# Aleph-Alpha/magma

Hardware: NVIDIA H100
Metric: image-caption samples/sec (fwd+bwd) (higher is better)
Workload: dtype bf16

## Files before the change

magma_b200/csrc/gemm.cu:

```cuda
#include <mutex>
#include <stdlib.h>

#include "gemm_common.cuh"

namespace mb200 {

template <int BN, bool A_MN, bool B_MN>
__global__ void __launch_bounds__(kThreads, 1)
gemm_wgmma_kernel(const __grid_constant__ CUtensorMap tmA, const __grid_constant__ CUtensorMap tmB,
                  const __grid_constant__ GemmKernelParams p) {
  using C_ = Cfg<BN>;
  constexpr int kStages = C_::kStages;

  extern __shared__ uint8_t smem_raw[];
  uint8_t* smem = reinterpret_cast<uint8_t*>((reinterpret_cast<uintptr_t>(smem_raw) + 1023) & ~uintptr_t(1023));
  uint8_t* smem_a = smem;
  uint8_t* smem_b = smem + kStages * C_::kABytes;
  float* epi_stage = reinterpret_cast<float*>(smem + kStages * C_::kStageBytes);
  uint64_t* full_bar = reinterpret_cast<uint64_t*>(smem + kStages * C_::kStageBytes + kEpiBytes);
  uint64_t* empty_bar = full_bar + kStages;

  const int wg = threadIdx.x >> 7;
  const int num_kb = (p.K + BK - 1) / BK;
  const int items = p.total_tiles * p.split_k;

  pdl_trigger();
  if (threadIdx.x == 0) {
    tma_prefetch_desc(&tmA);
    tma_prefetch_desc(&tmB);
    for (int s = 0; s < kStages; ++s) {
      mbar_init(&full_bar[s], 1);
      mbar_init(&empty_bar[s], 2);
    }
    mbar_fence_init();
  }
  __syncthreads();
  pdl_wait();

  if (wg == 0) {
    setmaxnreg_dec<40>();
    if (threadIdx.x == 0) {
      int stage = 0;
      uint32_t phase = 0;
      for (int w = blockIdx.x; w < items; w += gridDim.x) {
        const int t = w / p.split_k, ks = w - t * p.split_k;
        const int kb0 = ks * p.kb_per_split, kb1 = min(num_kb, kb0 + p.kb_per_split);
        const int tpb = p.tiles_m * p.tiles_n;
        const int z = t / tpb;
        const int r = t - z * tpb;
        const int m_blk = r % p.tiles_m;
        const int n_blk = r / p.tiles_m;
        const int z0 = z % p.nb0, z1 = z / p.nb0;
        for (int kb = kb0; kb < kb1; ++kb) {
          mbar_wait(&empty_bar[stage], phase ^ 1);
          mbar_expect_tx(&full_bar[stage], (uint32_t)C_::kStageBytes);
          uint8_t* sa = smem_a + stage * C_::kABytes;
          uint8_t* sb = smem_b + stage * C_::kBBytes;
          const int kc = kb * BK;
          if constexpr (A_MN) {
#pragma unroll
            for (int i = 0; i < BM / 64; ++i)
              tma_load_4d(sa + i * 8192, &tmA, &full_bar[stage], m_blk * BM + i * 64, kc, z0, z1);
          } else {
            tma_load_4d(sa, &tmA, &full_bar[stage], kc, m_blk * BM, z0, z1);
          }
          if constexpr (B_MN) {
#pragma unroll
            for (int i = 0; i < BN / 64; ++i)
              tma_load_4d(sb + i * 8192, &tmB, &full_bar[stage], n_blk * BN + i * 64, kc, z0, z1);
          } else {
            tma_load_4d(sb, &tmB, &full_bar[stage], kc, n_blk * BN, z0, z1);
          }
          if (++stage == kStages) {
            stage = 0;
            phase ^= 1;
          }
        }
      }
    }
  } else {
    setmaxnreg_inc<232>();
    const int cw = wg - 1;
    const bool leader = (threadIdx.x & 127) == 0;
    constexpr uint32_t b_lbo = B_MN ? 8192u : 0u;
    constexpr uint32_t a_kadv = A_MN ? 2048u : 32u, b_kadv = B_MN ? 2048u : 32u;
    const uint32_t a_off = (uint32_t)cw * 8192u;
    int stage = 0;
    uint32_t phase = 0;
    float acc[BN / 2];
    for (int w = blockIdx.x; w < items; w += gridDim.x) {
      const int t = w / p.split_k, ks = w - t * p.split_k;
      const int kb0 = ks * p.kb_per_split, kb1 = min(num_kb, kb0 + p.kb_per_split);
      const int tpb = p.tiles_m * p.tiles_n;
      const int z = t / tpb;
      const int r = t - z * tpb;
      const int m_blk = r % p.tiles_m;
      const int n_blk = r / p.tiles_m;
      const int z0 = z % p.nb0, z1 = z / p.nb0;
      int prev = -1;
      for (int kb = kb0; kb < kb1; ++kb) {
        mbar_wait(&full_bar[stage], phase);
        const uint32_t sa = smem_u32(smem_a + stage * C_::kABytes) + a_off;
        const uint32_t sb = smem_u32(smem_b + stage * C_::kBBytes);
        wgmma_fence();
#pragma unroll
        for (int k = 0; k < BK / WG_K; ++k) {
          const uint64_t da = make_smem_desc(sa + k * a_kadv, 0u, 1024);
          const uint64_t db = make_smem_desc(sb + k * b_kadv, b_lbo, 1024);
          wgmma_bf16<BN, A_MN ? 1 : 0, B_MN ? 1 : 0>(acc, da, db, (kb > kb0 || k > 0) ? 1u : 0u);
        }
        wgmma_commit();
        wgmma_wait<1>();
        if (prev >= 0 && leader) mbar_arrive(&empty_bar[prev]);
        prev = stage;
        if (++stage == kStages) {
          stage = 0;
          phase ^= 1;
        }
      }
      wgmma_wait<0>();
      if (prev >= 0 && leader) mbar_arrive(&empty_bar[prev]);
      const long long boff = (long long)z0 * p.c_bs0 + (long long)z1 * p.c_bs1;
      epi_tile<BN>(p, acc, epi_stage + cw * 64 * kEpiCols, 1 + cw, boff, m_blk * BM + cw * 64, n_blk * BN, ks);
    }
  }
}

__global__ void splitk_finalize_kernel(const GemmKernelParams p) {
  pdl_trigger();
  pdl_wait();
  const int ncol4 = (p.N + 3) >> 2;
  const long long total = (long long)p.M * ncol4;
  for (long long i = blockIdx.x * (long long)blockDim.x + threadIdx.x; i < total; i += (long long)gridDim.x * blockDim.x) {
    const int row = (int)(i / ncol4);
    const int col = (int)(i - (long long)row * ncol4) * 4;
    float v[4] = {0.f, 0.f, 0.f, 0.f};
    for (int ks = 0; ks < p.split_k; ++ks) {
      const float4 w4 = *reinterpret_cast<const float4*>(p.splitk_ws + ((long long)ks * p.M + row) * p.ld_ws + col);
      v[0] += w4.x;
      v[1] += w4.y;
      v[2] += w4.z;
      v[3] += w4.w;
    }
    epi_store4(p, 0, row, col, v);
  }
}

typedef CUresult (*PFN_encodeTiled)(CUtensorMap*, CUtensorMapDataType, cuuint32_t, void*, const cuuint64_t*,
                                    const cuuint64_t*, const cuuint32_t*, const cuuint32_t*, CUtensorMapInterleave,
                                    CUtensorMapSwizzle, CUtensorMapL2promotion, CUtensorMapFloatOOBfill);

static PFN_encodeTiled get_encode_fn() {
  static PFN_encodeTiled fn = nullptr;
  static std::once_flag once;
  std::call_once(once, [] {
    void* p = nullptr;
    cudaDriverEntryPointQueryResult qres;
    if (cudaGetDriverEntryPoint("cuTensorMapEncodeTiled", &p, cudaEnableDefault, &qres) == cudaSuccess &&
        qres == cudaDriverEntryPointSuccess)
      fn = reinterpret_cast<PFN_encodeTiled>(p);
  });
  return fn;
}

int make_operand_map(CUtensorMap* out, const mb200_operand& op, int rows, int K, int nb0, int nb1,
                            int box_rows) {
  PFN_encodeTiled enc = get_encode_fn();
  MB_REQUIRE(enc != nullptr, MB200_E_CUDA, "cuTensorMapEncodeTiled entry point unavailable");
  MB_REQUIRE((reinterpret_cast<uintptr_t>(op.ptr) & 15) == 0, MB200_E_ALIGN, "gemm operand pointer not 16B aligned");
  MB_REQUIRE(op.ld % 8 == 0, MB200_E_ALIGN, "gemm operand ld (%lld) must be a multiple of 8 elements",
             (long long)op.ld);
  MB_REQUIRE((nb0 == 1 || op.bs0 % 8 == 0) && (nb1 == 1 || op.bs1 % 8 == 0), MB200_E_ALIGN,
             "gemm operand batch strides must be multiples of 8 elements");
  cuuint64_t dims[4];
  cuuint64_t strides[3];
  cuuint32_t box[4];
  cuuint32_t estr[4] = {1, 1, 1, 1};
  if (!op.mn_major) {
    dims[0] = (cuuint64_t)K;
    dims[1] = (cuuint64_t)rows;
    box[0] = BK;
    box[1] = (cuuint32_t)box_rows;
  } else {
    dims[0] = (cuuint64_t)rows;
    dims[1] = (cuuint64_t)K;
    box[0] = 64;
    box[1] = BK;
  }
  dims[2] = (cuuint64_t)nb0;
  dims[3] = (cuuint64_t)nb1;
  box[2] = 1;
  box[3] = 1;
  strides[0] = (cuuint64_t)op.ld * 2;
  strides[1] = (cuuint64_t)(nb0 > 1 ? op.bs0 : op.ld) * 2;
  strides[2] = (cuuint64_t)(nb1 > 1 ? op.bs1 : op.ld) * 2;
  CUresult r = enc(out, CU_TENSOR_MAP_DATA_TYPE_BFLOAT16, 4, const_cast<void*>(op.ptr), dims, strides, box, estr,
                   CU_TENSOR_MAP_INTERLEAVE_NONE, CU_TENSOR_MAP_SWIZZLE_128B, CU_TENSOR_MAP_L2_PROMOTION_L2_256B,
                   CU_TENSOR_MAP_FLOAT_OOB_FILL_NONE);
  MB_REQUIRE(r == CUDA_SUCCESS, MB200_E_CUDA,
             "cuTensorMapEncodeTiled failed (%d): dims=(%llu,%llu,%llu,%llu) strides=(%llu,%llu,%llu) box=(%u,%u)",
             (int)r, (unsigned long long)dims[0], (unsigned long long)dims[1], (unsigned long long)dims[2],
             (unsigned long long)dims[3], (unsigned long long)strides[0], (unsigned long long)strides[1],
             (unsigned long long)strides[2], box[0], box[1]);
  return 0;
}

template <int BN, bool A_MN, bool B_MN>
static int launch_gemm(const CUtensorMap& tmA, const CUtensorMap& tmB, const GemmKernelParams& kp,
                       cudaStream_t stream) {
  auto kern = gemm_wgmma_kernel<BN, A_MN, B_MN>;
  static bool attr_set = false;
  if (!attr_set) {
    MB_CUDA(cudaFuncSetAttribute(kern, cudaFuncAttributeMaxDynamicSharedMemorySize, Cfg<BN>::kSmemBytes));
    attr_set = true;
  }
  const long long items = (long long)kp.total_tiles * kp.split_k;
  int grid = items < gemm_sms() ? (int)items : gemm_sms();
  {
    const double nb = (double)kp.total_tiles / ((double)kp.tiles_m * kp.tiles_n);
    const double flops = 2.0 * kp.M * (double)kp.N * kp.K * nb;
    const double bytes = nb * (2.0 * ((double)kp.M * kp.K + (double)kp.N * kp.K) + (kp.c_f32 ? 4.0 : 2.0) * kp.M * kp.N);
    GemmProfScope prof(stream, flops, bytes);
    MB_CUDA(launch_pdl(kern, dim3(grid), dim3(kThreads), Cfg<BN>::kSmemBytes, stream, tmA, tmB, kp));
  }
  count_launch();
  MB_CUDA(cudaGetLastError());
  return 0;
}

template <int BN>
static int dispatch_major(bool a_mn, bool b_mn, const CUtensorMap& tmA, const CUtensorMap& tmB,
                          const GemmKernelParams& kp, cudaStream_t s) {
  if (!a_mn && !b_mn) return launch_gemm<BN, false, false>(tmA, tmB, kp, s);
  if (!a_mn && b_mn) return launch_gemm<BN, false, true>(tmA, tmB, kp, s);
  if (a_mn && !b_mn) return launch_gemm<BN, true, false>(tmA, tmB, kp, s);
  return launch_gemm<BN, true, true>(tmA, tmB, kp, s);
}

static int dispatch_bn(int bn, bool a_mn, bool b_mn, const CUtensorMap& tmA, const CUtensorMap& tmB,
                       const GemmKernelParams& kp, cudaStream_t s) {
  switch (bn) {
    case 64: return dispatch_major<64>(a_mn, b_mn, tmA, tmB, kp, s);
    case 128: return dispatch_major<128>(a_mn, b_mn, tmA, tmB, kp, s);
    default: return dispatch_major<256>(a_mn, b_mn, tmA, tmB, kp, s);
  }
}

static int pick_bn(int M, int N, int batches) {
  if (N <= 64) return 64;
  const int tiles_m = (M + BM - 1) / BM;
  const int sms = num_sms();
  double best = 1e300;
  int best_bn = 256;
  const int cands[3] = {256, 128, 64};
  const double tile_cost[3] = {1.0, 0.55, 0.3};
  for (int i = 0; i < 3; ++i) {
    const int bn = cands[i];
    if (bn > 64 && N <= bn / 2) continue;
    const long long t = (long long)tiles_m * ((N + bn - 1) / bn) * batches;
    const long long waves = (t + sms - 1) / sms;
    const double cost = (double)waves * tile_cost[i];
    if (cost < best - 1e-12) {
      best = cost;
      best_bn = bn;
    }
  }
  return best_bn;
}

struct SmallPlan {
  int bn, split;
};
static SmallPlan plan_small_m(int N, int K, int M, size_t ws_bytes) {
  const int sms = num_sms();
  const int num_kb = (K + BK - 1) / BK;
  const double kHbmRate = 3.35e12, kItem = 4e-6, kFinalize = 4e-6;
  SmallPlan best{64, 1};
  double best_t = 1e300;
  const int cands[3] = {256, 128, 64};
  for (int i = 0; i < 3; ++i) {
    const int bn = cands[i];
    if (bn > 64 && N <= bn / 2) continue;
    const int tiles = (N + bn - 1) / bn;
    for (int split = 1; split <= 16; ++split) {
      if (split > 1) {
        if (num_kb / split < 8) break;
        if ((size_t)split * M * ((N + 3) / 4 * 4) * sizeof(float) > ws_bytes) break;
      }
      const int kb_per = (num_kb + split - 1) / split;
      const int eff_split = (num_kb + kb_per - 1) / kb_per;
      const long long items = (long long)tiles * eff_split;
      const long long waves = (items + sms - 1) / sms;
      const double active = (double)(items < sms ? items : sms);
      const double sm_rate = bn == 64 ? 40e9 : 50e9;
      const double rate = sm_rate < kHbmRate / active ? sm_rate : kHbmRate / active;
      const double t = kItem + waves * ((double)kb_per * bn * BK * 2 / rate) + (eff_split > 1 ? kFinalize : 0.0);
      if (t < best_t - 1e-12) {
        best_t = t;
        best = SmallPlan{bn, eff_split};
      }
    }
  }
  return best;
}

int gemm_impl(const mb200_gemm_args* a, cudaStream_t stream) {
  MB_REQUIRE(a != nullptr, MB200_E_ARG, "null gemm args");
  MB_REQUIRE(a->M > 0 && a->N > 0 && a->K > 0 && a->nb0 > 0 && a->nb1 > 0, MB200_E_SHAPE,
             "gemm: bad shape M=%d N=%d K=%d nb=(%d,%d)", a->M, a->N, a->K, a->nb0, a->nb1);
  MB_REQUIRE(a->c_dtype == MB200_BF16 || a->c_dtype == MB200_F32, MB200_E_DTYPE, "gemm: bad c_dtype %d", a->c_dtype);
  MB_REQUIRE(!(a->accumulate && a->c_dtype != MB200_F32), MB200_E_DTYPE, "gemm: accumulate needs f32 output");
  MB_REQUIRE(!(a->dact && !a->aux_in), MB200_E_ARG, "gemm: dact needs aux_in");
  const int celt = a->c_dtype == MB200_F32 ? 4 : 8;
  MB_REQUIRE((reinterpret_cast<uintptr_t>(a->C) & 15) == 0 && a->ldc % celt == 0, MB200_E_ALIGN,
             "gemm: C must be 16B aligned with ldc multiple of %d", celt);
  MB_REQUIRE((a->nb0 == 1 || a->c_bs0 % celt == 0) && (a->nb1 == 1 || a->c_bs1 % celt == 0), MB200_E_ALIGN,
             "gemm: C batch strides must be multiples of %d elements", celt);
  if (a->res1 || a->res2) MB_REQUIRE(a->ld_res % 8 == 0, MB200_E_ALIGN, "gemm: ld_res must be a multiple of 8");
  if (a->aux_in || a->aux_out)
    MB_REQUIRE(a->ldc % 8 == 0, MB200_E_ALIGN, "gemm: aux tensors share ldc, which must be a multiple of 8");
  int rc = check_arch();
  if (rc) return rc;

  int bn = a->force_bn ? a->force_bn : pick_bn(a->M, a->N, a->nb0 * a->nb1);
  MB_REQUIRE(bn == 64 || bn == 128 || bn == 256, MB200_E_ARG, "gemm: force_bn must be 64, 128 or 256");

  CUtensorMap tmA, tmB;
  const bool small_m = a->M <= 32 && a->A.mn_major == 0 && a->nb0 * a->nb1 == 1 && a->c_dtype == MB200_BF16;
  int plan_split = 1;
  if (small_m && !a->force_bn) {
    const SmallPlan pl = plan_small_m(a->N, a->K, a->M, a->splitk_ws ? (size_t)a->splitk_ws_bytes : 0);
    bn = pl.bn;
    plan_split = pl.split;
  }
  rc = make_operand_map(&tmA, a->A, a->M, a->K, a->nb0, a->nb1, BM);
  if (rc) return rc;

  GemmKernelParams kp;
  memset(&kp, 0, sizeof(kp));
  kp.M = a->M;
  kp.N = a->N;
  kp.K = a->K;
  kp.nb0 = a->nb0;
  kp.tiles_m = (a->M + BM - 1) / BM;
  kp.C = a->C;
  kp.ldc = a->ldc;
  kp.c_bs0 = a->c_bs0;
  kp.c_bs1 = a->c_bs1;
  kp.alpha = a->alpha;
  kp.act = a->act;
  kp.dact = a->dact;
  kp.accumulate = a->accumulate;
  kp.bias = reinterpret_cast<const bf16*>(a->bias);
  kp.aux_out = reinterpret_cast<bf16*>(a->aux_out);
  kp.aux_in = reinterpret_cast<const bf16*>(a->aux_in);
  kp.res1 = reinterpret_cast<const bf16*>(a->res1);
  kp.res2 = reinterpret_cast<const bf16*>(a->res2);
  kp.ld_res = a->ld_res;
  kp.epi_kind = EK_GENERIC;
  kp.c_f32 = a->c_dtype == MB200_F32 ? 1 : 0;
  kp.rope_tab = reinterpret_cast<const float2*>(a->rope_tab);
  kp.rope_mode = a->rope_tab ? a->rope_mode : 0;
  kp.rope_S = a->rope_S;
  kp.rope_hd = a->rope_hd;
  kp.rope_rot = a->rope_rot;
  kp.rope_ncols = a->rope_ncols;
  if (kp.rope_mode != 0)
    MB_REQUIRE(a->rope_S > 0 && a->rope_hd > 0 && a->rope_rot % 4 == 0 && a->rope_rot <= a->rope_hd &&
                   a->rope_hd % 4 == 0 && a->rope_ncols % 4 == 0,
               MB200_E_ARG, "gemm: bad rope epilogue parameters");

  const bool amn = a->A.mn_major != 0, bmn = a->B.mn_major != 0;
  kp.split_k = 1;
  kp.kb_per_split = (a->K + BK - 1) / BK;
  const bool split_mid = !small_m && a->splitk_ws && a->M <= 128 && a->nb0 * a->nb1 == 1 && a->K >= 8192 &&
                         a->N <= 8192 && !a->force_bn;
  const int bn_few = a->N >= 256 ? 256 : (a->N > 64 ? 128 : 64);
  const int tiles_m = kp.tiles_m;
  const bool split_few = !small_m && !split_mid && a->splitk_ws && a->M > 128 && a->nb0 * a->nb1 == 1 &&
                         a->K >= 2048 && !a->force_bn && 2 * tiles_m * ((a->N + bn_few - 1) / bn_few) <= num_sms();
  if (plan_split > 1 || split_mid || split_few) {
    const int bn_s = small_m ? bn : bn_few;
    const int tiles = (a->N + bn_s - 1) / bn_s;
    const int num_kb = (a->K + BK - 1) / BK;
    int split = plan_split;
    if (split_mid || split_few) {
      split = num_sms() / (tiles * tiles_m);
      if (split > num_kb / 4) split = num_kb / 4;
    }
    const long long ld_ws = (a->N + 3) / 4 * 4;
    while (split > 1 && (size_t)split * a->M * ld_ws * sizeof(float) > (size_t)a->splitk_ws_bytes) --split;
    if (split > 1) {
      const int kb_per = (num_kb + split - 1) / split;
      split = (num_kb + kb_per - 1) / kb_per;
      bn = bn_s;
      rc = make_operand_map(&tmB, a->B, a->N, a->K, a->nb0, a->nb1, bn);
      if (rc) return rc;
      kp.tiles_n = tiles;
      kp.total_tiles = tiles_m * tiles;
      kp.split_k = split;
      kp.kb_per_split = kb_per;
      kp.splitk_ws = reinterpret_cast<float*>(a->splitk_ws);
      kp.ld_ws = ld_ws;
      GemmKernelParams kg = kp;
      kg.epi_kind = EK_SPLITK;
      rc = dispatch_bn(bn, amn, bmn, tmA, tmB, kg, stream);
      if (rc) return rc;
      const long long n4 = (long long)a->M * ((a->N + 3) / 4);
      const int fgrid = (int)((n4 + 255) / 256 > 2048 ? 2048 : (n4 + 255) / 256);
      kp.alpha = 1.f;
      MB_CUDA(launch_pdl(splitk_finalize_kernel, dim3(fgrid), dim3(256), 0, stream, kp));
      count_launch();
      return 0;
    }
  }
  rc = make_operand_map(&tmB, a->B, a->N, a->K, a->nb0, a->nb1, bn);
  if (rc) return rc;
  kp.tiles_n = (a->N + bn - 1) / bn;
  kp.total_tiles = tiles_m * kp.tiles_n * a->nb0 * a->nb1;
  return dispatch_bn(bn, amn, bmn, tmA, tmB, kp, stream);
}

}

extern "C" int mb200_gemm(const mb200_gemm_args* args, void* stream) {
  return mb200::gemm_impl(args, reinterpret_cast<cudaStream_t>(stream));
}
```

magma_b200/csrc/gemm_common.cuh:

```cuda
#pragma once
#include "common.cuh"

namespace mb200 {

static constexpr int BM = 128;
static constexpr int BK = 64;
static constexpr int WG_K = 16;
static constexpr int kThreads = 384;
static constexpr int kEpiCols = 64;
static constexpr int kEpiBytes = BM * kEpiCols * 4;
static constexpr int kSmemBudget = 192 * 1024;

template <int BN>
struct Cfg {
  static constexpr int kABytes = BM * BK * 2;
  static constexpr int kBBytes = BN * BK * 2;
  static constexpr int kStageBytes = kABytes + kBBytes;
  static constexpr int kStagesRaw = kSmemBudget / kStageBytes;
  static constexpr int kStages = kStagesRaw > 8 ? 8 : kStagesRaw;
  static constexpr int kSmemBytes = kStages * kStageBytes + kEpiBytes + 1024  + 256 ;
  static_assert(kSmemBytes <= 227 * 1024, "GEMM shared memory exceeds the sm_90 per-block limit");
};

struct GemmKernelParams {
  int M, N, K;
  int nb0;
  int tiles_m, tiles_n, total_tiles;
  void* C;
  long long ldc, c_bs0, c_bs1;
  float alpha;
  int act, dact, accumulate;
  const bf16* bias;
  bf16* aux_out;
  const bf16* aux_in;
  const bf16* res1;
  const bf16* res2;
  long long ld_res;
  const float2* rope_tab;
  int rope_mode;
  int rope_S, rope_hd, rope_rot, rope_ncols;
  int epi_kind;
  int c_f32;
  int split_k, kb_per_split;
  float* splitk_ws;
  long long ld_ws;
};

__device__ __forceinline__ float2 bf16x2_to_f32(uint32_t u) {
  return __bfloat1622float2(*reinterpret_cast<const __nv_bfloat162*>(&u));
}
__device__ __forceinline__ uint32_t f32x2_to_bf16(float a, float b) {
  __nv_bfloat162 h = __floats2bfloat162_rn(a, b);
  return *reinterpret_cast<uint32_t*>(&h);
}

__device__ __forceinline__ void ld_bf16x4(const bf16* src, int n, float (&v)[4]) {
  if (n == 4 && (reinterpret_cast<uintptr_t>(src) & 7) == 0) {
    uint32_t u0, u1;
    asm volatile("ld.global.nc.v2.u32 {%0, %1}, [%2];" : "=r"(u0), "=r"(u1) : "l"(src));
    const float2 a = bf16x2_to_f32(u0), b = bf16x2_to_f32(u1);
    v[0] = a.x;
    v[1] = a.y;
    v[2] = b.x;
    v[3] = b.y;
  } else {
#pragma unroll
    for (int e = 0; e < 4; ++e) v[e] = e < n ? __bfloat162float(src[e]) : 0.f;
  }
}
__device__ __forceinline__ void st_bf16x4(bf16* dst, int n, const float (&v)[4]) {
  if (n == 4 && (reinterpret_cast<uintptr_t>(dst) & 7) == 0) {
    *reinterpret_cast<uint2*>(dst) = make_uint2(f32x2_to_bf16(v[0], v[1]), f32x2_to_bf16(v[2], v[3]));
  } else {
#pragma unroll
    for (int e = 0; e < 4; ++e)
      if (e < n) dst[e] = __float2bfloat16(v[e]);
  }
}

__device__ __forceinline__ void named_bar_sync(int id, int nthreads) {
  asm volatile("bar.sync %0, %1;" ::"r"(id), "r"(nthreads) : "memory");
}

enum { EK_GENERIC = 0, EK_SPLITK };

__device__ __forceinline__ void epi_store4(const GemmKernelParams& p, long long boff, int row, int col, float (&v)[4]) {
  const int n = min(4, p.N - col);
  if (p.bias) {
    float b[4];
    ld_bf16x4(p.bias + col, n, b);
#pragma unroll
    for (int e = 0; e < 4; ++e) v[e] += b[e];
  }
  if (p.rope_mode != 0 && col < p.rope_ncols) {
    const int dim = col % p.rope_hd;
    if (dim < p.rope_rot) {
      const float2* tp = p.rope_tab + (long long)(row % p.rope_S) * (p.rope_rot >> 1) + (dim >> 1);
      const float2 cs0 = __ldg(tp), cs1 = __ldg(tp + 1);
      const float sg = p.rope_mode > 0 ? 1.f : -1.f;
      const float a0 = v[0], a1 = v[1], a2 = v[2], a3 = v[3];
      v[0] = a0 * cs0.x - a1 * cs0.y * sg;
      v[1] = a1 * cs0.x + a0 * cs0.y * sg;
      v[2] = a2 * cs1.x - a3 * cs1.y * sg;
      v[3] = a3 * cs1.x + a2 * cs1.y * sg;
    }
  }
  const long long coff = boff + (long long)row * p.ldc + col;
  if (p.aux_out) st_bf16x4(p.aux_out + coff, n, v);
#pragma unroll
  for (int e = 0; e < 4; ++e) {
    if (p.act == MB200_ACT_GELU_NEW) v[e] = gelu_new_f(v[e]);
    else if (p.act == MB200_ACT_QUICK_GELU) v[e] = quick_gelu_f(v[e]);
    else if (p.act == MB200_ACT_RELU) v[e] = fmaxf(v[e], 0.f);
  }
  if (p.dact) {
    float a[4];
    ld_bf16x4(p.aux_in + coff, n, a);
#pragma unroll
    for (int e = 0; e < 4; ++e) v[e] = p.dact == MB200_DACT_GELU_NEW ? v[e] * gelu_new_grad_f(a[e]) : (a[e] > 0.f ? v[e] : 0.f);
  }
  const long long roff = boff + (long long)row * p.ld_res + col;
  if (p.res1) {
    float r[4];
    ld_bf16x4(p.res1 + roff, n, r);
#pragma unroll
    for (int e = 0; e < 4; ++e) v[e] += r[e];
  }
  if (p.res2) {
    float r[4];
    ld_bf16x4(p.res2 + roff, n, r);
#pragma unroll
    for (int e = 0; e < 4; ++e) v[e] += r[e];
  }
  if (p.act == MB200_ACT_RELU_POST) {
#pragma unroll
    for (int e = 0; e < 4; ++e) v[e] = fmaxf(v[e], 0.f);
  }
  if (p.c_f32) {
    float* dst = reinterpret_cast<float*>(p.C) + coff;
    if (n == 4) {
      float4 o = make_float4(v[0], v[1], v[2], v[3]);
      if (p.accumulate) {
        const float4 old = *reinterpret_cast<const float4*>(dst);
        o.x += old.x;
        o.y += old.y;
        o.z += old.z;
        o.w += old.w;
      }
      *reinterpret_cast<float4*>(dst) = o;
    } else {
#pragma unroll
      for (int e = 0; e < 4; ++e)
        if (e < n) dst[e] = p.accumulate ? dst[e] + v[e] : v[e];
    }
  } else {
    st_bf16x4(reinterpret_cast<bf16*>(p.C) + coff, n, v);
  }
}

template <int BN>
__device__ __forceinline__ void epi_tile(const GemmKernelParams& p, const float (&acc)[BN / 2], float* stage,
                                         int bar_id, long long boff, int row0, int col0, int ks) {
  const int wt = threadIdx.x & 127;
  const int fr = (wt >> 5) * 16 + ((wt & 31) >> 2);
  const int fq = wt & 3;
  const int pr = wt >> 4, pc = wt & 15;
  const int nch = min(BN / kEpiCols, (p.N - col0 + kEpiCols - 1) / kEpiCols);
#pragma unroll 1
  for (int ch = 0; ch < nch; ++ch) {
#pragma unroll
    for (int c = 0; c < BN / kEpiCols; ++c) {
      if (c != ch) continue;
#pragma unroll
      for (int jj = 0; jj < 8; ++jj) {
        const int j = c * 8 + jj;
#pragma unroll
        for (int h = 0; h < 2; ++h) {
          const int r = fr + 8 * h;
          const int q = (2 * jj + (fq >> 1)) ^ ((r & 3) << 1);
          *reinterpret_cast<float2*>(stage + r * kEpiCols + q * 4 + 2 * (fq & 1)) =
              make_float2(acc[4 * j + 2 * h], acc[4 * j + 2 * h + 1]);
        }
      }
    }
    named_bar_sync(bar_id, 128);
    const int col = col0 + ch * kEpiCols + pc * 4;
#pragma unroll 1
    for (int i = 0; i < 64 / 8; ++i) {
      const int r = pr + 8 * i;
      const int row = row0 + r;
      if (row >= p.M || col >= p.N) continue;
      const float4 s = *reinterpret_cast<const float4*>(stage + r * kEpiCols + ((pc ^ ((r & 3) << 1)) * 4));
      float v[4] = {s.x * p.alpha, s.y * p.alpha, s.z * p.alpha, s.w * p.alpha};
      if (p.epi_kind == EK_SPLITK) {
        *reinterpret_cast<float4*>(p.splitk_ws + ((long long)ks * p.M + row) * p.ld_ws + col) =
            make_float4(v[0], v[1], v[2], v[3]);
        continue;
      }
      epi_store4(p, boff, row, col, v);
    }
    named_bar_sync(bar_id, 128);
  }
}

int make_operand_map(CUtensorMap* out, const mb200_operand& op, int rows, int K, int nb0, int nb1, int box_rows);

}
```

Baseline: 128.9.

## Prefetch epilogue residual/aux inputs via TMA through the operand smem ring

Adds TMA tensor maps for the epilogue inputs (dact aux, residual 1/2). The producer warp queues these tiles into the existing operand pipeline stages after each tile's K loop, and the consumer epilogue reads them from shared memory instead of issuing scattered global loads per row. Bias loads are hoisted out of the per-row loop. This adds a kernel template variant, extra barrier handshakes on the ring, and alignment preconditions, with a fallback to the old global-load path.

```diff
diff --git a/magma_b200/csrc/gemm.cu b/magma_b200/csrc/gemm.cu
--- a/magma_b200/csrc/gemm.cu
+++ b/magma_b200/csrc/gemm.cu
@@ -5,10 +5,17 @@
 
 namespace mb200 {
 
-template <int BN, bool A_MN, bool B_MN>
+template <bool kOn>
+struct EpiMaps {
+  CUtensorMap m[3];
+};
+template <>
+struct EpiMaps<false> {};
+
+template <int BN, bool A_MN, bool B_MN, bool EPI_TMA>
 __global__ void __launch_bounds__(kThreads, 1)
 gemm_wgmma_kernel(const __grid_constant__ CUtensorMap tmA, const __grid_constant__ CUtensorMap tmB,
-                  const __grid_constant__ GemmKernelParams p) {
+                  const __grid_constant__ EpiMaps<EPI_TMA> tmE, const __grid_constant__ GemmKernelParams p) {
   using C_ = Cfg<BN>;
   constexpr int kStages = C_::kStages;
 
@@ -19,6 +26,7 @@
   float* epi_stage = reinterpret_cast<float*>(smem + kStages * C_::kStageBytes);
   uint64_t* full_bar = reinterpret_cast<uint64_t*>(smem + kStages * C_::kStageBytes + kEpiBytes);
   uint64_t* empty_bar = full_bar + kStages;
+  const EpiRing ring{smem_a, smem_b, full_bar, empty_bar};
 
   const int wg = threadIdx.x >> 7;
   const int num_kb = (p.K + BK - 1) / BK;
@@ -28,6 +36,10 @@
   if (threadIdx.x == 0) {
     tma_prefetch_desc(&tmA);
     tma_prefetch_desc(&tmB);
+    if constexpr (EPI_TMA) {
+#pragma unroll 1
+      for (int i = 0; i < p.epi_in; ++i) tma_prefetch_desc(&tmE.m[i]);
+    }
     for (int s = 0; s < kStages; ++s) {
       mbar_init(&full_bar[s], 1);
       mbar_init(&empty_bar[s], 2);
@@ -76,6 +88,7 @@
             phase ^= 1;
           }
         }
+        if constexpr (EPI_TMA) epi_queue_inputs<BN>(p, tmE.m, ring, stage, phase, m_blk * BM, n_blk * BN, z0, z1);
       }
     }
   } else {
@@ -121,7 +134,8 @@
       wgmma_wait<0>();
       if (prev >= 0 && leader) mbar_arrive(&empty_bar[prev]);
       const long long boff = (long long)z0 * p.c_bs0 + (long long)z1 * p.c_bs1;
-      epi_tile<BN>(p, acc, epi_stage + cw * 64 * kEpiCols, 1 + cw, boff, m_blk * BM + cw * 64, n_blk * BN, ks);
+      epi_tile<BN, EPI_TMA>(p, acc, epi_stage + cw * 64 * kEpiCols, 1 + cw, boff, m_blk * BM + cw * 64, n_blk * BN, ks, ring,
+                   stage, phase);
     }
   }
 }
@@ -142,7 +156,10 @@
       v[2] += w4.z;
       v[3] += w4.w;
     }
-    epi_store4(p, 0, row, col, v);
+    EpiIn in;
+    if (p.bias) ld_bf16x4(p.bias + col, min(4, p.N - col), in.bias);
+    epi_load_inputs(p, 0, row, col, in);
+    epi_store4(p, 0, row, col, v, in);
   }
 }
 
@@ -205,10 +222,10 @@
   return 0;
 }
 
-template <int BN, bool A_MN, bool B_MN>
-static int launch_gemm(const CUtensorMap& tmA, const CUtensorMap& tmB, const GemmKernelParams& kp,
-                       cudaStream_t stream) {
-  auto kern = gemm_wgmma_kernel<BN, A_MN, B_MN>;
+template <int BN, bool A_MN, bool B_MN, bool EPI_TMA>
+static int launch_gemm(const CUtensorMap& tmA, const CUtensorMap& tmB, const EpiMaps<true>& tmE,
+                       const GemmKernelParams& kp, cudaStream_t stream) {
+  auto kern = gemm_wgmma_kernel<BN, A_MN, B_MN, EPI_TMA>;
   static bool attr_set = false;
   if (!attr_set) {
     MB_CUDA(cudaFuncSetAttribute(kern, cudaFuncAttributeMaxDynamicSharedMemorySize, Cfg<BN>::kSmemBytes));
@@ -221,29 +238,72 @@
     const double flops = 2.0 * kp.M * (double)kp.N * kp.K * nb;
     const double bytes = nb * (2.0 * ((double)kp.M * kp.K + (double)kp.N * kp.K) + (kp.c_f32 ? 4.0 : 2.0) * kp.M * kp.N);
     GemmProfScope prof(stream, flops, bytes);
-    MB_CUDA(launch_pdl(kern, dim3(grid), dim3(kThreads), Cfg<BN>::kSmemBytes, stream, tmA, tmB, kp));
+    if constexpr (EPI_TMA)
+      MB_CUDA(launch_pdl(kern, dim3(grid), dim3(kThreads), Cfg<BN>::kSmemBytes, stream, tmA, tmB, tmE, kp));
+    else
+      MB_CUDA(launch_pdl(kern, dim3(grid), dim3(kThreads), Cfg<BN>::kSmemBytes, stream, tmA, tmB, EpiMaps<false>{}, kp));
   }
   count_launch();
   MB_CUDA(cudaGetLastError());
   return 0;
 }
 
-template <int BN>
+template <int BN, bool EPI_TMA>
 static int dispatch_major(bool a_mn, bool b_mn, const CUtensorMap& tmA, const CUtensorMap& tmB,
-                          const GemmKernelParams& kp, cudaStream_t s) {
-  if (!a_mn && !b_mn) return launch_gemm<BN, false, false>(tmA, tmB, kp, s);
-  if (!a_mn && b_mn) return launch_gemm<BN, false, true>(tmA, tmB, kp, s);
-  if (a_mn && !b_mn) return launch_gemm<BN, true, false>(tmA, tmB, kp, s);
-  return launch_gemm<BN, true, true>(tmA, tmB, kp, s);
+                          const EpiMaps<true>& tmE, const GemmKernelParams& kp, cudaStream_t s) {
+  if (!a_mn && !b_mn) return launch_gemm<BN, false, false, EPI_TMA>(tmA, tmB, tmE, kp, s);
+  if (!a_mn && b_mn) return launch_gemm<BN, false, true, EPI_TMA>(tmA, tmB, tmE, kp, s);
+  if (a_mn && !b_mn) return launch_gemm<BN, true, false, EPI_TMA>(tmA, tmB, tmE, kp, s);
+  return launch_gemm<BN, true, true, EPI_TMA>(tmA, tmB, tmE, kp, s);
 }
 
 static int dispatch_bn(int bn, bool a_mn, bool b_mn, const CUtensorMap& tmA, const CUtensorMap& tmB,
-                       const GemmKernelParams& kp, cudaStream_t s) {
+                       const EpiMaps<true>& tmE, const GemmKernelParams& kp, cudaStream_t s) {
+  const bool epi = kp.epi_in != 0;
   switch (bn) {
-    case 64: return dispatch_major<64>(a_mn, b_mn, tmA, tmB, kp, s);
-    case 128: return dispatch_major<128>(a_mn, b_mn, tmA, tmB, kp, s);
-    default: return dispatch_major<256>(a_mn, b_mn, tmA, tmB, kp, s);
-  }
+    case 64:
+      return epi ? dispatch_major<64, true>(a_mn, b_mn, tmA, tmB, tmE, kp, s)
+                 : dispatch_major<64, false>(a_mn, b_mn, tmA, tmB, tmE, kp, s);
+    case 128:
+      return epi ? dispatch_major<128, true>(a_mn, b_mn, tmA, tmB, tmE, kp, s)
+                 : dispatch_major<128, false>(a_mn, b_mn, tmA, tmB, tmE, kp, s);
+    default:
+      return epi ? dispatch_major<256, true>(a_mn, b_mn, tmA, tmB, tmE, kp, s)
+                 : dispatch_major<256, false>(a_mn, b_mn, tmA, tmB, tmE, kp, s);
+  }
+}
+
+static int make_epi_maps(EpiMaps<true>* maps, GemmKernelParams* kp, const mb200_gemm_args* a) {
+  const void* ptr[3];
+  long long ld[3];
+  int n = 0;
+  if (a->dact) {
+    ptr[n] = a->aux_in;
+    ld[n++] = a->ldc;
+  }
+  if (a->res1) {
+    ptr[n] = a->res1;
+    ld[n++] = a->ld_res;
+  }
+  if (a->res2) {
+    ptr[n] = a->res2;
+    ld[n++] = a->ld_res;
+  }
+  bool ok = (a->nb0 == 1 || a->c_bs0 % 8 == 0) && (a->nb1 == 1 || a->c_bs1 % 8 == 0);
+  for (int i = 0; i < n; ++i) ok = ok && (reinterpret_cast<uintptr_t>(ptr[i]) & 15) == 0 && ld[i] % 8 == 0;
+  if (n == 0 || !ok) return 0;
+  for (int i = 0; i < n; ++i) {
+    mb200_operand op;
+    memset(&op, 0, sizeof(op));
+    op.ptr = ptr[i];
+    op.ld = ld[i];
+    op.bs0 = a->c_bs0;
+    op.bs1 = a->c_bs1;
+    const int rc = make_operand_map(&maps->m[i], op, a->M, a->N, a->nb0, a->nb1, BM);
+    if (rc) return rc;
+  }
+  kp->epi_in = n;
+  return 0;
 }
 
 static int pick_bn(int M, int N, int batches) {
@@ -326,6 +386,8 @@
   MB_REQUIRE(bn == 64 || bn == 128 || bn == 256, MB200_E_ARG, "gemm: force_bn must be 64, 128 or 256");
 
   CUtensorMap tmA, tmB;
+  EpiMaps<true> tmE;
+  memset(&tmE, 0, sizeof(tmE));
   const bool small_m = a->M <= 32 && a->A.mn_major == 0 && a->nb0 * a->nb1 == 1 && a->c_dtype == MB200_BF16;
   int plan_split = 1;
   if (small_m && !a->force_bn) {
@@ -404,7 +466,7 @@
       kp.ld_ws = ld_ws;
       GemmKernelParams kg = kp;
       kg.epi_kind = EK_SPLITK;
-      rc = dispatch_bn(bn, amn, bmn, tmA, tmB, kg, stream);
+      rc = dispatch_bn(bn, amn, bmn, tmA, tmB, tmE, kg, stream);
       if (rc) return rc;
       const long long n4 = (long long)a->M * ((a->N + 3) / 4);
       const int fgrid = (int)((n4 + 255) / 256 > 2048 ? 2048 : (n4 + 255) / 256);
@@ -418,7 +480,9 @@
   if (rc) return rc;
   kp.tiles_n = (a->N + bn - 1) / bn;
   kp.total_tiles = tiles_m * kp.tiles_n * a->nb0 * a->nb1;
-  return dispatch_bn(bn, amn, bmn, tmA, tmB, kp, stream);
+  rc = make_epi_maps(&tmE, &kp, a);
+  if (rc) return rc;
+  return dispatch_bn(bn, amn, bmn, tmA, tmB, tmE, kp, stream);
 }
 
 }
diff --git a/magma_b200/csrc/gemm_common.cuh b/magma_b200/csrc/gemm_common.cuh
--- a/magma_b200/csrc/gemm_common.cuh
+++ b/magma_b200/csrc/gemm_common.cuh
@@ -9,6 +9,7 @@
 static constexpr int kThreads = 384;
 static constexpr int kEpiCols = 64;
 static constexpr int kEpiBytes = BM * kEpiCols * 4;
+static constexpr int kEpiBoxBytes = BM * kEpiCols * 2;
 static constexpr int kSmemBudget = 192 * 1024;
 
 template <int BN>
@@ -20,6 +21,9 @@
   static constexpr int kStages = kStagesRaw > 8 ? 8 : kStagesRaw;
   static constexpr int kSmemBytes = kStages * kStageBytes + kEpiBytes + 1024  + 256 ;
   static_assert(kSmemBytes <= 227 * 1024, "GEMM shared memory exceeds the sm_90 per-block limit");
+  static constexpr int kEpiBoxesPerStage = 1 + kBBytes / kEpiBoxBytes;
+  static_assert(kABytes == kEpiBoxBytes && kEpiBoxesPerStage * kEpiBoxBytes <= kStageBytes, "epilogue box layout");
+  static_assert(3 * (BN / kEpiCols) <= kStages * kEpiBoxesPerStage, "epilogue inputs exceed the operand ring");
 };
 
 struct GemmKernelParams {
@@ -36,6 +40,7 @@
   const bf16* res1;
   const bf16* res2;
   long long ld_res;
+  int epi_in;
   const float2* rope_tab;
   int rope_mode;
   int rope_S, rope_hd, rope_rot, rope_ncols;
@@ -84,13 +89,34 @@
 
 enum { EK_GENERIC = 0, EK_SPLITK };
 
-__device__ __forceinline__ void epi_store4(const GemmKernelParams& p, long long boff, int row, int col, float (&v)[4]) {
+struct EpiIn {
+  float bias[4], aux[4], res1[4], res2[4];
+};
+
+__device__ __forceinline__ void epi_load_inputs(const GemmKernelParams& p, long long boff, int row, int col,
+                                                EpiIn& in) {
+  const int n = min(4, p.N - col);
+  if (p.dact) ld_bf16x4(p.aux_in + boff + (long long)row * p.ldc + col, n, in.aux);
+  const long long roff = boff + (long long)row * p.ld_res + col;
+  if (p.res1) ld_bf16x4(p.res1 + roff, n, in.res1);
+  if (p.res2) ld_bf16x4(p.res2 + roff, n, in.res2);
+}
+
+__device__ __forceinline__ void ld_smem_bf16x4(const uint8_t* src, float (&v)[4]) {
+  const uint2 u = *reinterpret_cast<const uint2*>(src);
+  const float2 a = bf16x2_to_f32(u.x), b = bf16x2_to_f32(u.y);
+  v[0] = a.x;
+  v[1] = a.y;
+  v[2] = b.x;
+  v[3] = b.y;
+}
+
+__device__ __forceinline__ void epi_store4(const GemmKernelParams& p, long long boff, int row, int col, float (&v)[4],
+                                           const EpiIn& in) {
   const int n = min(4, p.N - col);
   if (p.bias) {
-    float b[4];
-    ld_bf16x4(p.bias + col, n, b);
-#pragma unroll
-    for (int e = 0; e < 4; ++e) v[e] += b[e];
+#pragma unroll
+    for (int e = 0; e < 4; ++e) v[e] += in.bias[e];
   }
   if (p.rope_mode != 0 && col < p.rope_ncols) {
     const int dim = col % p.rope_hd;
@@ -114,23 +140,17 @@
     else if (p.act == MB200_ACT_RELU) v[e] = fmaxf(v[e], 0.f);
   }
   if (p.dact) {
-    float a[4];
-    ld_bf16x4(p.aux_in + coff, n, a);
-#pragma unroll
-    for (int e = 0; e < 4; ++e) v[e] = p.dact == MB200_DACT_GELU_NEW ? v[e] * gelu_new_grad_f(a[e]) : (a[e] > 0.f ? v[e] : 0.f);
-  }
-  const long long roff = boff + (long long)row * p.ld_res + col;
+#pragma unroll
+    for (int e = 0; e < 4; ++e)
+      v[e] = p.dact == MB200_DACT_GELU_NEW ? v[e] * gelu_new_grad_f(in.aux[e]) : (in.aux[e] > 0.f ? v[e] : 0.f);
+  }
   if (p.res1) {
-    float r[4];
-    ld_bf16x4(p.res1 + roff, n, r);
-#pragma unroll
-    for (int e = 0; e < 4; ++e) v[e] += r[e];
+#pragma unroll
+    for (int e = 0; e < 4; ++e) v[e] += in.res1[e];
   }
   if (p.res2) {
-    float r[4];
-    ld_bf16x4(p.res2 + roff, n, r);
-#pragma unroll
-    for (int e = 0; e < 4; ++e) v[e] += r[e];
+#pragma unroll
+    for (int e = 0; e < 4; ++e) v[e] += in.res2[e];
   }
   if (p.act == MB200_ACT_RELU_POST) {
 #pragma unroll
@@ -158,14 +178,50 @@
   }
 }
 
+
+struct EpiRing {
+  uint8_t* a;
+  uint8_t* b;
+  uint64_t* full;
+  uint64_t* empty;
+};
+
 template <int BN>
+__device__ __forceinline__ int epi_chunks(const GemmKernelParams& p, int col0) {
+  return min(BN / kEpiCols, (p.N - col0 + kEpiCols - 1) / kEpiCols);
+}
+
+template <int BN>
+__device__ __forceinline__ uint8_t* epi_box(const EpiRing& ring, int s, int k) {
+  return k == 0 ? ring.a + s * Cfg<BN>::kABytes : ring.b + s * Cfg<BN>::kBBytes + (k - 1) * kEpiBoxBytes;
+}
+
+template <int BN, bool EPI_TMA>
 __device__ __forceinline__ void epi_tile(const GemmKernelParams& p, const float (&acc)[BN / 2], float* stage,
-                                         int bar_id, long long boff, int row0, int col0, int ks) {
+                                         int bar_id, long long boff, int row0, int col0, int ks, const EpiRing& ring,
+                                         int& ring_stage, uint32_t& ring_phase) {
+  constexpr int kStages = Cfg<BN>::kStages, kBps = Cfg<BN>::kEpiBoxesPerStage;
   const int wt = threadIdx.x & 127;
   const int fr = (wt >> 5) * 16 + ((wt & 31) >> 2);
   const int fq = wt & 3;
   const int pr = wt >> 4, pc = wt & 15;
-  const int nch = min(BN / kEpiCols, (p.N - col0 + kEpiCols - 1) / kEpiCols);
+  const int nch = epi_chunks<BN>(p, col0);
+  const int nin = EPI_TMA ? p.epi_in : 0;
+  int bs = ring_stage, bk = 0, rs = ring_stage;
+  uint32_t bph = ring_phase;
+  auto next_box = [&]() {
+    if (bk == 0) mbar_wait(&ring.full[bs], bph);
+    const uint8_t* box = epi_box<BN>(ring, bs, bk);
+    if (++bk == kBps) {
+      bk = 0;
+      if (++bs == kStages) {
+        bs = 0;
+        bph ^= 1;
+      }
+    }
+    return box;
+  };
+  const int box_off = ((row0 % BM) + pr) * 128 + (((pc >> 1) ^ pr) << 4) + ((pc & 1) << 3);
 #pragma unroll 1
   for (int ch = 0; ch < nch; ++ch) {
 #pragma unroll
@@ -185,6 +241,14 @@
     }
     named_bar_sync(bar_id, 128);
     const int col = col0 + ch * kEpiCols + pc * 4;
+    const uint8_t *src_aux = nullptr, *src_res1 = nullptr, *src_res2 = nullptr;
+    if (nin) {
+      if (p.dact) src_aux = next_box() + box_off;
+      if (p.res1) src_res1 = next_box() + box_off;
+      if (p.res2) src_res2 = next_box() + box_off;
+    }
+    EpiIn in;
+    if (p.bias && col < p.N) ld_bf16x4(p.bias + col, min(4, p.N - col), in.bias);
 #pragma unroll 1
     for (int i = 0; i < 64 / 8; ++i) {
       const int r = pr + 8 * i;
@@ -197,9 +261,57 @@
             make_float4(v[0], v[1], v[2], v[3]);
         continue;
       }
-      epi_store4(p, boff, row, col, v);
+      if (nin) {
+        if (p.dact) ld_smem_bf16x4(src_aux + i * 1024, in.aux);
+        if (p.res1) ld_smem_bf16x4(src_res1 + i * 1024, in.res1);
+        if (p.res2) ld_smem_bf16x4(src_res2 + i * 1024, in.res2);
+      } else {
+        epi_load_inputs(p, boff, row, col, in);
+      }
+      epi_store4(p, boff, row, col, v, in);
     }
     named_bar_sync(bar_id, 128);
+    if (nin) {
+      if (ch + 1 == nch && bk != 0) {
+        bk = 0;
+        if (++bs == kStages) {
+          bs = 0;
+          bph ^= 1;
+        }
+      }
+#pragma unroll 1
+      for (; rs != bs; rs = rs + 1 == kStages ? 0 : rs + 1)
+        if (wt == 0) mbar_arrive(&ring.empty[rs]);
+    }
+  }
+  ring_stage = bs;
+  ring_phase = bph;
+}
+
+template <int BN>
+__device__ __forceinline__ void epi_queue_inputs(const GemmKernelParams& p, const CUtensorMap* maps,
+                                                 const EpiRing& ring, int& stage, uint32_t& phase, int m0, int col0,
+                                                 int z0, int z1) {
+  constexpr int kStages = Cfg<BN>::kStages, kBps = Cfg<BN>::kEpiBoxesPerStage;
+  const int nbox = p.epi_in * epi_chunks<BN>(p, col0);
+  int col = col0, i = 0;
+#pragma unroll 1
+  for (int b0 = 0; b0 < nbox; b0 += kBps) {
+    const int nb = min(kBps, nbox - b0);
+    mbar_wait(&ring.empty[stage], phase ^ 1);
+    mbar_expect_tx(&ring.full[stage], (uint32_t)(nb * kEpiBoxBytes));
+#pragma unroll 1
+    for (int k = 0; k < nb; ++k) {
+      tma_load_4d(epi_box<BN>(ring, stage, k), &maps[i], &ring.full[stage], col, m0, z0, z1);
+      if (++i == p.epi_in) {
+        i = 0;
+        col += kEpiCols;
+      }
+    }
+    if (++stage == kStages) {
+      stage = 0;
+      phase ^= 1;
+    }
   }
 }
 
```

After: 135.5 (median of 6 runs). +5.1%, better.
